# finlaymiller/torch-vae

Hardware: AMD Instinct MI355X
Metric: training samples/sec (VAE step: forward+ELBO+backward+AdamW), synthetic pianoroll (higher is better)
Workload: dtype bf16; 1 GPU; VanillaVAE latent_dim=16, 128x128 synthetic pianoroll, batch 256/GPU (generalised bottleneck 256*(H/16)^2); img_size=128, latent_dim=16, batch_per_gpu=256, global_batch=256, parallelism=dp1, optimizer=AdamW+OneCycle (encoder, decoder groups)

## Files before the change

### torch_vae_amd/csrc/conv_mfma.cuh

```cuda
#pragma once
#include "common.cuh"

enum { EPI_FWD = 0, EPI_BWD = 1, EPI_PLAIN = 2 };

template <typename T> struct ConvArgs {
    const T* src0; const T* src1; const float* coef; float slope;
    const T* wp; const float* bias;
    T* out;
    const T* yout; const float* ocoef; float oslope;
    double* stat;
    int B, Hs, Ws, Cin, Cout;
    int lth, ltw, lTB, tiles_x, tiles_y;
    int two_src, epi;
    unsigned m_pp, m_pw, m_tx, m_txy;
    long long* dbg;
    BnFuse fuse;
    int rev, n_mt;
    int xcd;
    T* stage_out;
};

__device__ __forceinline__ int fastdiv(int x, unsigned m) { return m ? (int)__umulhi((unsigned)x, m) : x; }
static inline unsigned fastdiv_magic(int d) { return d <= 1 ? 0u : (unsigned)((0x100000000ULL + (unsigned long long)d - 1) / (unsigned long long)d); }

// ... 1079 lines not shown
    sdl = wave_sum(sdl); bsum = wave_sum(bsum);
    __syncthreads();
    if (r < 9) {
#pragma unroll
        for (int i = 0; i < 16; ++i) red[wave][r * 32 + acc_row(i, lane)] = accw[i];
    }
    if (h == 0) { red[wave][288 + r] = s1; red[wave][320 + r] = s2; }
    if (lane == 0) { red[wave][352] = sdl; red[wave][353] = bsum; }
    __syncthreads();
    for (int j = tid; j < 288; j += 256) a.slab[(size_t)blockIdx.x * 288 + j] = red[0][j] + red[1][j] + red[2][j] + red[3][j];
    if (tid < 64) unsafeAtomicAdd(&a.stat[stat_rep() * 64 + tid], (double)(red[0][288 + tid] + red[1][288 + tid] + red[2][288 + tid] + red[3][288 + tid]));
    if (tid == 64) unsafeAtomicAdd(&a.accum[stat_rep() * 8 + 2], (double)(red[0][352] + red[1][352] + red[2][352] + red[3][352]));
    if (tid == 65) unsafeAtomicAdd(&a.accum[stat_rep() * 8 + 0], (double)(red[0][353] + red[1][353] + red[2][353] + red[3][353]));
}

template <typename T> struct DenseArgs {
    const T* A; const float* coef; float slope; int C;
    const T* Bp;
    float* slab;
    int M, K, Npad, ksteps_per_split;
    BnFuse fuse;
};

template <typename T, int NT>
__global__ __launch_bounds__(256) void dense_kernel(DenseArgs<T> a) {
    const int tid = threadIdx.x, lane = tid & 63, wave = tid >> 6, r = lane & 31, h = lane >> 5;
    const int m = blockIdx.x * 128 + wave * 32 + r, n0 = blockIdx.z * 32 * NT;
    const int ks0 = blockIdx.y * a.ksteps_per_split, ks1 = min(a.K / 16, ks0 + a.ksteps_per_split);
    __shared__ float dcf[2 * 256];
    if (a.coef) {
        const bool writer = blockIdx.x == 0 && blockIdx.y == 0 && blockIdx.z == 0;
        for (int c = tid; c < a.C; c += 256) {
            if (a.fuse.mode == BNF_FWD) { float k1; bn_fused_channel(a.fuse, c, writer, dcf[c], k1, dcf[256 + c]); }
            else { dcf[c] = a.coef[c]; dcf[256 + c] = a.coef[2 * a.C + c]; }
        }
        __syncthreads();
    }
    f32x16 acc[NT];
#pragma unroll
    for (int nt = 0; nt < NT; ++nt)
#pragma unroll
        for (int i = 0; i < 16; ++i) acc[nt][i] = 0.f;
    for (int ks = ks0; ks < ks1; ++ks) {
        const int k = ks * 16 + 8 * h;
        Frag<T> af;
        if (m < a.M) {
            Frag<T> raw = load_frag(a.A + (size_t)m * a.K + k);
            if (a.coef) {
#pragma unroll
                for (int j = 0; j < 8; ++j) {
                    const int c = (k + j) & (a.C - 1);
                    float v;
                    if constexpr (sizeof(T) == 4) v = raw.v[j]; else v = (float)raw.v[j];
                    af.set(j, leaky(v * dcf[c] + dcf[256 + c], a.slope));
                }
            } else {
                af = raw;
            }
        } else {
#pragma unroll
            for (int j = 0; j < 8; ++j) af.set(j, 0.f);
        }
#pragma unroll
        for (int nt = 0; nt < NT; ++nt) {
            const int n = n0 + nt * 32 + r;
            Frag<T> bf = load_frag(a.Bp + ((size_t)(k >> 3) * a.Npad + (n < a.Npad ? n : 0)) * 8);
            mma(acc[nt], af, bf);
        }
    }
#pragma unroll
    for (int nt = 0; nt < NT; ++nt)
#pragma unroll
        for (int i = 0; i < 16; ++i) {
            const int mm = blockIdx.x * 128 + wave * 32 + acc_row(i, lane), n = n0 + nt * 32 + r;
            if (mm < a.M && n < a.Npad) a.slab[((size_t)blockIdx.y * a.M + mm) * a.Npad + n] = acc[nt][i];
        }
}
```

### torch_vae_amd/csrc/edge_kernels.cuh

```cuda
#pragma once
#include "common.cuh"

__device__ __forceinline__ float cg_sum(float v) {
#pragma unroll
    for (int o = 4; o < 64; o <<= 1) v += __shfl_xor(v, o, 64);
    return v;
}

template <typename T> __device__ __forceinline__ void load8(const T* p, float* o);
template <> __device__ __forceinline__ void load8<float>(const float* p, float* o) {
    f32x4 a = *reinterpret_cast<const f32x4*>(p), b = *reinterpret_cast<const f32x4*>(p + 4);
#pragma unroll
    for (int i = 0; i < 4; ++i) { o[i] = a[i]; o[4 + i] = b[i]; }
}
template <> __device__ __forceinline__ void load8<bf16>(const bf16* p, float* o) {
    bf16x8 a = *reinterpret_cast<const bf16x8*>(p);
#pragma unroll
    for (int i = 0; i < 8; ++i) o[i] = (float)a[i];
}
template <> __device__ __forceinline__ void load8<f16>(const f16* p, float* o) {
    f16x8 a = *reinterpret_cast<const f16x8*>(p);
#pragma unroll
    for (int i = 0; i < 8; ++i) o[i] = (float)a[i];
}
// ... 750 lines not shown
#pragma unroll
            for (int u = 0; u < 8; ++u)
                av[u] = (bb + u < nb) ? leaky(tofloat(a.y[(size_t)(bc + bb + u) * a.F + fp]) * sc + sh, a.slope) : 0.f;
#pragma unroll
            for (int u = 0; u < 8; ++u)
#pragma unroll
                for (int q = 0; q < JT / 4; ++q) {
                    const f32x4 d = *reinterpret_cast<const f32x4*>(&dl_s[(bb + u) * JT + q * 4]);
#pragma unroll
                    for (int e = 0; e < 4; ++e) acc[q * 4 + e] += d[e] * av[u];
                }
        }
    }
#pragma unroll
    for (int j = 0; j < JT; ++j) {
        const int jj = j0 + j;
        const size_t zoff = (size_t)blockIdx.z * a.L * a.F;
        if (jj < a.L) a.dwmu[zoff + (size_t)jj * a.F + fr] = acc[j];
        else if (jj < L2) a.dwvar[zoff + (size_t)(jj - a.L) * a.F + fr] = acc[j];
    }
}

constexpr int DECIN_LC = 512;
static inline size_t decin_fwd_lds(int L) { return (size_t)16 * std::min(L, DECIN_LC) * 4; }
template <typename T>
__global__ __launch_bounds__(256) void decin_fwd_kernel(const float* __restrict__ z, const float* __restrict__ wd,
                                                        const float* __restrict__ bd, T* __restrict__ d0, int B, int F, int L, int s2) {
    constexpr int BT = 16;
    extern __shared__ __attribute__((aligned(16))) float z_s[];
    const int tid = threadIdx.x, fp = blockIdx.x * 256 + tid, b0 = blockIdx.y * BT, fr = fref_of(fp, s2);
    float acc[BT];
    const float bias = bd[fr];
#pragma unroll
    for (int bb = 0; bb < BT; ++bb) acc[bb] = bias;
    const float* wrow = wd + (size_t)fr * L;
    for (int l0 = 0; l0 < L; l0 += DECIN_LC) {
        const int nl = min(DECIN_LC, L - l0);
        if (l0) __syncthreads();
        for (int i = tid; i < BT * nl; i += 256) {
            const int bb = i / nl, l = i - bb * nl;
            z_s[i] = (b0 + bb < B) ? z[(size_t)(b0 + bb) * L + l0 + l] : 0.f;
        }
        __syncthreads();
        if ((L & 3) == 0) {
            for (int l = 0; l < nl; l += 4) {
                const f32x4 w = *reinterpret_cast<const f32x4*>(wrow + l0 + l);
#pragma unroll
                for (int bb = 0; bb < BT; ++bb) {
                    const f32x4 zz = *reinterpret_cast<const f32x4*>(&z_s[bb * nl + l]);
                    acc[bb] += zz[0] * w[0] + zz[1] * w[1] + zz[2] * w[2] + zz[3] * w[3];
                }
            }
        } else {
            for (int l = 0; l < nl; ++l) {
                const float w = wrow[l0 + l];
#pragma unroll
                for (int bb = 0; bb < BT; ++bb) acc[bb] += z_s[bb * nl + l] * w;
            }
        }
    }
#pragma unroll
    for (int bb = 0; bb < BT; ++bb)
        if (b0 + bb < B) d0[(size_t)(b0 + bb) * F + fp] = fromfloat<T>(acc[bb]);
}

template <typename T>
__global__ __launch_bounds__(256) void decin_wgrad_kernel(const T* __restrict__ dd0, const float* __restrict__ z,
                                                          float* __restrict__ dwd, float* __restrict__ dbd, int B, int F, int L, int s2,
                                                          int bsplit) {
    constexpr int LT = 32, BC = 64;
    __shared__ __attribute__((aligned(16))) float z_s[BC * LT];
    const int tid = threadIdx.x, l0 = blockIdx.y * LT;
    int fp, fr;
    fmap_ref_major(blockIdx.x, tid, s2, fp, fr);
    float acc[LT], sb = 0.f;
#pragma unroll
    for (int l = 0; l < LT; ++l) acc[l] = 0.f;
    const int bz0 = blockIdx.z * bsplit, bz1 = min(B, bz0 + bsplit);
    for (int bc = bz0; bc < bz1; bc += BC) {
        __syncthreads();
        for (int i = tid; i < BC * LT; i += 256) {
            const int bb = i / LT, l = i % LT;
            z_s[i] = (bc + bb < bz1 && l0 + l < L) ? z[(size_t)(bc + bb) * L + l0 + l] : 0.f;
        }
        __syncthreads();
        const int nb = min(BC, bz1 - bc);
// ... 137 lines not shown
```

### torch_vae_amd/csrc/latent_mfma.cuh

```cuda
#pragma once
#include "common.cuh"

struct FeatTile {
    int P, lP, CW, pix0, c0, s2;
    __device__ __forceinline__ FeatTile(int blk, int s2_) : s2(s2_) {
        P = s2_ < 8 ? s2_ : 8; lP = 31 - __clz(P); CW = 64 >> lP;
        const int lpb = (31 - __clz(s2_)) - lP;
        const int cblk = blk >> lpb; pix0 = (blk - (cblk << lpb)) << lP; c0 = cblk * CW;
    }
    __device__ __forceinline__ int fp(int col) const { return (pix0 + (col & (P - 1))) * 256 + c0 + (col >> lP); }
    __device__ __forceinline__ int fref(int col) const { return (c0 + (col >> lP)) * s2 + pix0 + (col & (P - 1)); }
    __device__ __forceinline__ int chan(int col) const { return c0 + (col >> lP); }
};

template <typename T>
__device__ __forceinline__ void stage_feat_tile_f32(const T* __restrict__ X, const FeatTile& t, int b0, int B, int F, const float* __restrict__ coef,
                                                    float slope, float* xs, int tid) {
    constexpr int E = 16 / sizeof(T);
    constexpr int vpr = 64 / E;
    const int lgpp = (6 - t.lP) - (E == 8 ? 3 : 2);
    for (int v = tid; v < 256 * vpr; v += 256) {
        const int row = v / vpr, j = v - row * vpr, p = j >> lgpp, g = j - (p << lgpp);
        const int b = b0 + row;
        float o[E];
        if (b < B) {
            const Vec16<T> raw = *reinterpret_cast<const Vec16<T>*>(X + (size_t)b * F + (t.pix0 + p) * 256 + t.c0 + g * E);
#pragma unroll
            for (int e = 0; e < E; ++e) {
                float x = raw.get(e);
                if (coef) { const int c = t.c0 + g * E + e; x = leaky(x * coef[c] + coef[2 * 256 + c], slope); }
                o[e] = x;
            }
        } else {
#pragma unroll
            for (int e = 0; e < E; ++e) o[e] = 0.f;
        }
#pragma unroll
        for (int e = 0; e < E; ++e) xs[row * 64 + (g * E + e) * t.P + p] = o[e];
    }
}

struct BatchGemmArgs {
    const void* X; const float* coef; float slope;
    const float* Y; int ldy, ncols;
    int ones_col;
    float* out0; float* out1; float* outb;
    float* colsum0; float* colsum1;
    int B, F, L, s2; float scale;
};

template <typename T, bool TRANSPOSED>
__global__ __launch_bounds__(256) void batch_gemm_kernel(BatchGemmArgs a) {
    constexpr int NBMAX = 9;
    extern __shared__ __attribute__((aligned(16))) char smem[];
    float* xs = reinterpret_cast<float*>(smem);
    float* ys = xs + 256 * 64;
    const int tid = threadIdx.x, lane = tid & 63, wave = tid >> 6, r = lane & 31, h = lane >> 5;
    const int fblk = wave & 1, khalf = wave >> 1;
    const FeatTile t(blockIdx.x, a.s2);
    const int ntot = a.ncols + (a.ones_col ? 1 : 0), nblk = (ntot + 31) / 32;
    f32x16 acc[NBMAX];
#pragma unroll
    for (int nb = 0; nb < NBMAX; ++nb)
#pragma unroll
        for (int i = 0; i < 16; ++i) acc[nb][i] = 0.f;
    for (int b0 = 0; b0 < a.B; b0 += 256) {
        __syncthreads();
        stage_feat_tile_f32<T>(reinterpret_cast<const T*>(a.X), t, b0, a.B, a.F, a.coef, a.slope, xs, tid);
#pragma unroll
        for (int nb = 0; nb < NBMAX; ++nb) {
            if (nb < nblk) {
                __syncthreads();
                if ((a.ldy & 3) == 0 && (a.ncols & 3) == 0) {
                    for (int i = tid; i < 256 * 8; i += 256) {
                        const int row = i >> 3, nq = (i & 7) * 4, n = nb * 32 + nq, b = b0 + row;
                        f32x4 v = {0.f, 0.f, 0.f, 0.f};
                        if (b < a.B) {
                            if (n < a.ncols) v = *reinterpret_cast<const f32x4*>(a.Y + (size_t)b * a.ldy + n);
                            else if (a.ones_col && n == a.ncols) v[0] = 1.f;
                        }
                        *reinterpret_cast<f32x4*>(ys + row * 32 + nq) = v;
                    }
                } else {
                    for (int i = tid; i < 256 * 32; i += 256) {
                        const int row = i >> 5, n = nb * 32 + (i & 31), b = b0 + row;
                        float v = 0.f;
                        if (b < a.B) v = n < a.ncols ? a.Y[(size_t)b * a.ldy + n] : ((a.ones_col && n == a.ncols) ? 1.f : 0.f);
                        ys[i] = v;
                    }
                }
                __syncthreads();
                if (blockIdx.x == 0 && a.colsum0) {
                    float s = 0.f;
                    for (int row = tid >> 5; row < 256; row += 8) s += ys[row * 32 + (tid & 31)];
                    float* cs = ys + 256 * 32;
                    cs[tid] = s;
                    __syncthreads();
                    const int n = nb * 32 + tid;
                    if (tid < 32 && n < a.ncols) {
                        float v = 0.f;
#pragma unroll
                        for (int g = 0; g < 8; ++g) v += cs[g * 32 + tid];
                        float* dst = n < a.L ? a.colsum0 + n : a.colsum1 + (n - a.L);
                        *dst = (b0 == 0 ? 0.f : *dst) + v * a.scale;
                    }
                }
                const float* xp = xs + (khalf * 128 + h) * 64 + fblk * 32 + r;
                const float* yp = ys + (khalf * 128 + h) * 32 + r;
#pragma unroll 8
                for (int s = 0; s < 64; ++s) {
                    const float xv = xp[s * 2 * 64], yv = yp[s * 2 * 32];
                    if constexpr (TRANSPOSED) acc[nb] = __builtin_amdgcn_mfma_f32_32x32x2f32(yv, xv, acc[nb], 0, 0, 0);
                    else acc[nb] = __builtin_amdgcn_mfma_f32_32x32x2f32(xv, yv, acc[nb], 0, 0, 0);
                }
// ... 11 lines not shown
    if (khalf == 0) {
#pragma unroll
        for (int nb = 0; nb < NBMAX; ++nb) {
            if (nb < nblk) {
#pragma unroll
                for (int i = 0; i < 16; ++i) {
                    const float v = (acc[nb][i] + red[((fblk * NBMAX + nb) * 16 + i) * 64 + lane]) * a.scale;
                    if constexpr (TRANSPOSED) {
                        const int n = nb * 32 + acc_row(i, lane), col = fblk * 32 + r;
                        if (n < a.ncols) {
                            float* dst = n < a.L ? a.out0 + (size_t)n * a.F : a.out1 + (size_t)(n - a.L) * a.F;
                            dst[t.fref(col)] = v;
                        }
                    } else {
                        const int col = fblk * 32 + acc_row(i, lane), n = nb * 32 + r;
                        if (n < a.ncols) a.out0[(size_t)t.fref(col) * a.L + n] = v;
                        else if (a.ones_col && n == a.ncols) a.outb[t.fref(col)] = v;
                    }
                }
            }
        }
    }
}
static inline size_t batch_gemm_lds() { return (size_t)(256 * 64 + 256 * 32 + 8 * 32) * 4; }

struct RowGemmArgs {
    const float* Y; int ldy, K;
    const float* Wf; const void* Wp; int npad;
    const float* bias;
    void* out;
    const void* y; const float* ocoef; float slope;
    const float* gpre; float gmul;
    double* stat;
    int B, F, s2;
};

template <typename T, int EPI>
__global__ __launch_bounds__(256) void row_gemm_kernel(RowGemmArgs a) {
    constexpr int KC = 32, YP = KC + 1;
    constexpr int E = 16 / sizeof(T);
    extern __shared__ __attribute__((aligned(16))) char smem[];
    float* ws = reinterpret_cast<float*>(smem);
    float* ys = ws + KC * 64;
    T* ot = reinterpret_cast<T*>(ys + 256 * YP);
    float* sred = reinterpret_cast<float*>(ot + 256 * 64);
    const int tid = threadIdx.x, lane = tid & 63, wave = tid >> 6, r = lane & 31, h = lane >> 5;
// ... 116 lines not shown
```

### torch_vae_amd/csrc/vae_api.hip

```cpp
#include <map>
#include <mutex>
#include "vae_ctx.h"
#include "edge_kernels.cuh"
#include "loglik.cuh"
#include "grad_clip.cuh"
#include "total_corr.cuh"

static thread_local std::string g_err;
int vae_set_error(const char* what, const char* why) {
    g_err = std::string(what) + ": " + why;
    return -1;
}

extern "C" const char* vae_last_error(void) { return g_err.c_str(); }
extern "C" int vae_abi_version(void) { return 1; }

static void param_shapes(int H, int L, int gen, int64_t* sizes) {
    const int s = gen ? H / 16 : 2;
    const int64_t F = 256LL * s * s;
    const int enc_ci[4] = {1, 32, 64, 128}, enc_co[4] = {32, 64, 128, 256};
    int k = 0;
    for (int i = 0; i < 4; ++i) { sizes[k++] = 9LL * enc_ci[i] * enc_co[i]; sizes[k++] = enc_co[i]; sizes[k++] = enc_co[i]; sizes[k++] = enc_co[i]; }
    sizes[k++] = L * F; sizes[k++] = L; sizes[k++] = L * F; sizes[k++] = L; sizes[k++] = F * L; sizes[k++] = F;
    const int dec_ci[3] = {256, 128, 64}, dec_co[3] = {128, 64, 32};
// ... 58 lines not shown
        (void)hipStreamSynchronize(c->comm);
        for (int i = 0; i < vae_ctx::NFORK; ++i) (void)hipEventDestroy(c->ev_fork[i]);
        (void)hipEventDestroy(c->ev_pack); (void)hipEventDestroy(c->ev_comm);
        if (c->ev_kl) (void)hipEventDestroy(c->ev_kl);
        for (int i = 0; i < vae_ctx::NBUCKET; ++i) (void)hipEventDestroy(c->ev_bucket[i]);
    }
    delete c;
}
extern "C" int64_t vae_workspace_bytes(const vae_ctx* c) { return c ? c->ws_bytes : 0; }

struct OptionDef { const char* name; int& (*ref)(vae_ctx&); int def; int (*norm)(int); };
static int opt_any(int v) { return v; }
static int opt_min1(int v) { return std::max(1, v); }
static int opt_fused_grid(int v) { return std::max(1, std::min(v, 512)); }
static int opt_max1024(int v) { return std::min(v, 1024); }
static int opt_max48(int v) { return std::min(v, 48); }
static int opt_fused_wgrad(int v) { return v == 1 ? 3 : v == 2 ? 1 : v == 3 ? 2 : 0; }
#define OPT(member, def, norm) {#member, [](vae_ctx& c) -> int& { return c.member; }, def, norm}
#define OPT_WK(member, def, norm) {"knob_wgrad_" #member, [](vae_ctx& c) -> int& { return c.wk.member; }, def, norm}
static const OptionDef kOptions[] = {
    OPT(use_tr16, 1, opt_any), OPT(use_mfma_convout, 1, opt_any), OPT(use_pipelined, 1, opt_any), OPT(use_side_stream, 1, opt_any),
    OPT(use_fused_bn, 1, opt_any), OPT(use_fused_convout, 1, opt_any), OPT(use_fused_wgrad, 1, opt_fused_wgrad), OPT(use_recomp_dz, 0, opt_any),
    OPT(use_raw_wgrad, 0, opt_any), OPT(use_deep, 1, opt_any), OPT(use_latent_mfma, 6, opt_any), OPT(use_convout_stream, 1, opt_any),
    OPT(use_dnf_stream, 1, opt_any), OPT(use_upf_stream, 1, opt_any), OPT(use_fc_dgrad8, 1, opt_any), OPT(use_wgrad_split, 1, opt_any),
    OPT(knob_up_per_cu, 2, opt_any), OPT(knob_down_per_cu, 2, opt_min1), OPT(knob_bwd_per_cu, 0, opt_any), OPT(knob_nt_max, 4, opt_any),
    OPT(knob_up_nt_max, 1, opt_min1), OPT(knob_wave_nt_max, 4, opt_any), OPT(knob_lay22_min_nt, 2, opt_any), OPT(knob_lay42, 1, opt_any),
    OPT(knob_down_waves, 8, opt_any), OPT(knob_pipe_max_cout, 256, opt_any), OPT(knob_xcd_map, 1, opt_any), OPT(knob_rev, 4, opt_any),
    OPT(knob_lean, 1, opt_any), OPT(knob_pack_grid, 128, opt_min1), OPT(knob_conv1_grid, 512, opt_any), OPT(knob_fused_grid, 256, opt_fused_grid),
    OPT(knob_convout_grid, 1536, opt_any), OPT(knob_convout_bwd_grid, 1024, opt_any), OPT(knob_convout_step_grid, 1024, opt_min1),
    OPT(knob_convout_bands, 0, opt_any), OPT(knob_wgrad_layer_wgs, 0, opt_any), OPT(knob_skip_wgrad, 0, opt_any), OPT(knob_ablate_b, 0, opt_any),
    OPT(knob_ablate_f, 0, opt_any),
    OPT_WK(tile, 1, opt_any), OPT_WK(wide, 1, opt_any), OPT_WK(mid8, 0, opt_any), OPT_WK(force_simple, 0, opt_any),
    OPT_WK(wgs, 128, opt_max1024), OPT_WK(wide_wgs, 128, opt_max1024), OPT_WK(cap_mb, 48, opt_max48),
};
#undef OPT_WK
#undef OPT
static const OptionDef* find_option(const char* name) {
    for (const OptionDef& o : kOptions) if (name && !strcmp(name, o.name)) return &o;
    return nullptr;
}

extern "C" vae_ctx* vae_create(int H, int L, int maxB, int dtype, int gen) {
    vae_ctx* c = new vae_ctx();
    c->H = H; c->L = L; c->maxB = maxB; c->dtype = dtype; c->gen = gen;
    for (const OptionDef& o : kOptions) o.ref(*c) = o.norm(o.def);
    if (getenv("VAE_NO_SIDE_STREAM")) c->use_side_stream = 0;
    if (vae_param_layout(H, L, gen, c->poff, c->psz, &c->ptotal) != 0) { delete c; return nullptr; }
// ... 777 lines not shown
```

### torch_vae_amd/csrc/vae_ctx.h

```cpp
#pragma once
#include <hip/hip_runtime.h>
#include <stdio.h>
#include <string.h>
#include <math.h>
#include <string>
#include <vector>
#include <algorithm>
#include <type_traits>

#include "../../include/vae_step.h"

int vae_set_error(const char* what, const char* why);

#include "common.cuh"

#define LAUNCH_CHECK(name)                                                        \
    do {                                                                          \
        hipError_t _e = hipGetLastError();                                        \
        if (_e != hipSuccess) return vae_set_error(name, hipGetErrorString(_e)); \
    } while (0)

template <typename K, typename... Args>
static int launch(const char* name, K kernel, dim3 grid, dim3 block, size_t lds_bytes, hipStream_t st, const Args&... args) {
    if (lds_bytes > 160 * 1024) return vae_set_error("lds", "tile needs more than 160 KiB LDS");
// ... 84 lines not shown
    PackDesc* d_descs; std::vector<PackDesc> h_descs; const float* packed_for = nullptr;
    float* slab; size_t slab_floats;
    static constexpr int NSIDE = 3, NFORK = 16;
    hipStream_t side[NSIDE]; float* side_slab[NSIDE]; hipEvent_t ev_fork[NFORK], ev_join[NSIDE], ev_pack; int side_rr = 0, fork_rr = 0, n_side_ok = 0;
    static constexpr int NBUCKET = 2; hipEvent_t ev_bucket[NBUCKET];
    hipStream_t comm; hipEvent_t ev_comm; int comm_busy = 0;
    void* nccl_comm = nullptr; int comm_rank = 0, comm_world = 0;
    double* dstats; size_t n_dstats; double* accum;
    float* reduce_tmp = nullptr; size_t reduce_tmp_floats = 0; unsigned reduce_slot = 0;
    float* fused_slab[3] = {nullptr, nullptr, nullptr}; size_t fused_slab_floats = 0;
    static constexpr int KL_SIDE = 2;
    void* kl_ws = nullptr; unsigned* kl_tk = nullptr; hipEvent_t ev_kl = nullptr;
    unsigned long long* kl_d() const { return static_cast<unsigned long long*>(kl_ws); }
    double* kl_scal() const { return reinterpret_cast<double*>(kl_d() + L); }
    float* kl_factor() const { return reinterpret_cast<float*>(kl_scal() + 2); }
    const double* kl_shaped() const { return fwd.kl_kind != VAE_KL_PLAIN ? kl_scal() : nullptr; }
    void* tc_ws = nullptr; size_t tc_ws_bytes = 0; int tc_ws_B = 0;
    float* tc_grad() const { return static_cast<float*>(tc_ws); }
    double* ps_part = nullptr; int ps_tb = 0, ps_ntile = 0;
    float* ll_f = nullptr; double* ll_part = nullptr; double* ll_lat = nullptr;
    double* ll_kb = nullptr; size_t ll_kb_n = 0;
    std::vector<void*> allocs; int64_t ws_bytes = 0;
    int use_tr16, use_mfma_convout, use_pipelined, use_side_stream, use_fused_bn, use_fused_convout, use_fused_wgrad, use_recomp_dz, use_raw_wgrad,
        use_deep, use_latent_mfma, use_convout_stream, use_dnf_stream, use_upf_stream, use_fc_dgrad8, use_wgrad_split;
    int knob_up_per_cu, knob_down_per_cu, knob_bwd_per_cu, knob_nt_max, knob_up_nt_max, knob_wave_nt_max, knob_lay22_min_nt, knob_lay42,
        knob_down_waves, knob_pipe_max_cout, knob_xcd_map, knob_rev, knob_lean, knob_pack_grid, knob_conv1_grid, knob_fused_grid,
        knob_convout_grid, knob_convout_bwd_grid, knob_convout_step_grid, knob_convout_bands, knob_wgrad_layer_wgs,
        knob_skip_wgrad, knob_ablate_b, knob_ablate_f;
    WgradKnobs wk;
    int recon = VAE_RECON_BCE, kl_kind = VAE_KL_PLAIN; double kl_param = 0.0; double recon_param = 0.0;
    FwdRecord fwd;
    long long* dbg_buf = nullptr; char dbg_tag[32] = {0}; int dbg_epi = 0;
    int prof = 0; const char* tag = nullptr; struct ProfRec { std::string name; hipEvent_t e0, e1; double bytes, flops; int side; int launches = 1; }; std::vector<ProfRec> prof_recs;
    hipStream_t cur_stream = nullptr; bool cur_stream_set = false;
};

struct ProfScope {
    vae_ctx* c; hipStream_t st; int idx;
    ProfScope(vae_ctx* c_, const char* name, double bytes, double flops, hipStream_t st_) : c(c_), st(st_), idx(-1) {
        if (!c || !c->prof) return;
        vae_ctx::ProfRec r; r.name = std::string(name) + (c->tag ? std::string(" @") + c->tag : std::string()); r.bytes = bytes; r.flops = flops;
        r.side = (c->cur_stream_set && st != c->cur_stream) ? 1 : 0;
        if (hipEventCreate(&r.e0) != hipSuccess || hipEventCreate(&r.e1) != hipSuccess) return;
        (void)hipEventRecord(r.e0, st);
        c->prof_recs.push_back(r); idx = (int)c->prof_recs.size() - 1;
    }
    ~ProfScope() { if (idx >= 0) (void)hipEventRecord(c->prof_recs[idx].e1, st); }
// ... 95 lines not shown
```

### torch_vae_amd/csrc/vae_impl.cuh

```cuda
#pragma once
#include "vae_ctx.h"
#include "conv_mfma.cuh"
#include "conv_pipe.cuh"
#include "edge_kernels.cuh"
#include "conv_fused.cuh"
#include "conv_deep.cuh"
#include "latent_mfma.cuh"
#include "convout_stream.cuh"
#include "wgrad_split.cuh"
#include "upfinal_stream.cuh"
#include "dnfirst_stream.cuh"
#include "grad_paths.cuh"

template <typename F> static int pick_recon(vae_ctx* c, F&& f) {
    return pick_const<VAE_RECON_BCE, VAE_RECON_MSE, VAE_RECON_WBCE>("reconstruction term", c->fwd.recon, f);
}
template <typename F> static int pick_recon_per_sample(vae_ctx* c, F&& f) {
    return pick_const<VAE_RECON_BCE, VAE_RECON_MSE>("reconstruction term", c->fwd.recon == VAE_RECON_WBCE ? VAE_RECON_BCE : c->fwd.recon, f);
}

static int stream_bands(int B, int rows, int max_bands, int min_rows, int rows_per_tick, int fixed_ticks) {
    const int ncu = 256;
    long best = -1; int nb = 1;
    for (int cand = 1; cand <= max_bands && rows / cand >= min_rows; cand *= 2) {
// ... 234 lines not shown
                a.dbg = (c->dbg_buf && c->tag && !strcmp(c->tag, c->dbg_tag) && c->dbg_epi == 32) ? c->dbg_buf : nullptr;
                rc = pick_bool(convt, [&](auto C) { return go(wgrad_split_kernel<T, decltype(C)::value>, 1024, wgrad_split_lds<T>(npix)); });
            }
            else if (WA == 4 && raw) rc = go(wgrad_kernel<T, 4, 1, false, true, 8, true>, 512, lds);
            else if (WA == 4) rc = pick_bool(convt, [&](auto C) { return go(wgrad_kernel<T, 4, 1, decltype(C)::value, true, 8>, 512, lds); });
            else rc = pick_bool(convt, [&](auto C) { return go(wgrad_kernel<T, 2, 1, decltype(C)::value, true, 8>, 512, lds); });
        }
        else rc = vae_set_error("wgrad", "eight-wave tiles need 16-bit storage");
    }
    else {
        const auto tile = [&](auto A, auto B_) { return pick_bool(convt, [&](auto C) { return pick_bool(pre, [&](auto P) {
            return go(wgrad_kernel<T, decltype(A)::value, decltype(B_)::value, decltype(C)::value, decltype(P)::value>, 256, lds); }); }); };
        using one = std::integral_constant<int, 1>; using two = std::integral_constant<int, 2>;
        if (WA == 2 && WB == 2) rc = tile(two{}, two{});
        else if (WA == 2 && WB == 1) rc = tile(two{}, one{});
        else if (WA == 1 && WB == 1) rc = tile(one{}, one{});
        else rc = vae_set_error("wgrad", "no kernel variant for this channel tile");
    }
    if (rc) return -1;
    }
    return launch_reduce(slab_buf, nsplit, (size_t)9 * a.CA * a.CB, dw_out, a.CA, a.CB, st, c);
}

template <typename T>
static int launch_dense(vae_ctx* c, DenseArgs<T> a, int* nsplit_out, hipStream_t st) {
    const int nb = a.Npad / 32, NT = nb % 4 == 0 ? 4 : (nb % 2 == 0 ? 2 : 1);
    if (a.Npad % 32) return vae_set_error("dense", "Npad must be a multiple of 32");
    const int mt = (a.M + 127) / 128, ntile = a.Npad / (32 * NT), ksteps = a.K / 16;
    int nsplit = std::max(1, std::min(ksteps, 512 / std::max(1, mt * ntile)));
    a.ksteps_per_split = (ksteps + nsplit - 1) / nsplit;
    nsplit = (ksteps + a.ksteps_per_split - 1) / a.ksteps_per_split;
    if ((size_t)nsplit * a.M * a.Npad > c->slab_floats) return vae_set_error("dense", "slab too small");
    a.slab = c->slab;
    dim3 grid(mt, nsplit, ntile);
    *nsplit_out = nsplit;
    ProfScope ps(c, "dense(fc / decoder_input dgrad)", sizeof(T) * ((double)a.M * a.K + (double)a.K * a.Npad), 2.0 * a.M * a.K * a.Npad, st);
    return pick_const<1, 2, 4>("dense_kernel", NT, [&](auto N) { return launch("dense_kernel", dense_kernel<T, decltype(N)::value>, grid, dim3(256), 0, st, a); });
}
template <typename T>
int pack_weights(vae_ctx* c, const float* params, hipStream_t st) {
    std::vector<PackDesc>& d = c->h_descs;
    if (c->packed_for != params || d.empty()) {
        d.clear();
        const int ci[8] = {1, 32, 64, 128, 256, 128, 64, 32}, co[8] = {32, 64, 128, 256, 128, 64, 32, 32};
        for (int i = 1; i < 8; ++i) {
            const bool conv = i < 4;
            PackDesc p; memset(&p, 0, sizeof(p));
            p.src = params + c->poff[c->lay[i].p_convw]; p.kind = 0; p.n = 9L * ci[i] * co[i];
            p.A = conv ? co[i] : ci[i]; p.Bc = conv ? ci[i] : co[i];
            p.dst = c->wp_fwd[i]; p.k_is_first = conv ? 0 : 1; d.push_back(p);
            p.dst = c->wp_dg[i]; p.k_is_first = conv ? 1 : 0; d.push_back(p);
        }
        PackDesc p; memset(&p, 0, sizeof(p));
        p.kind = 1; p.src = params + c->poff[16]; p.src2 = params + c->poff[18]; p.dst = c->fcpack; p.npad = c->npad_fc; p.L = c->L; p.s2 = c->s2; p.n = c->F * c->npad_fc; d.push_back(p);
        p.kind = 2; p.src = params + c->poff[20]; p.src2 = nullptr; p.dst = c->dipack; p.npad = c->npad_di; p.n = c->F * c->npad_di; d.push_back(p);
        p.kind = 3; p.src = params + c->poff[38]; p.dst = c->wout_t; p.A = 32; p.n = 288; d.push_back(p);
        HIP_CHECK_RET(hipMemcpyAsync(c->d_descs, d.data(), d.size() * sizeof(PackDesc), hipMemcpyHostToDevice, st));
        c->packed_for = params;
    }
    ProfScope ps(c, "pack_weights", 0, 0, st);
// ... 67 lines not shown
            c->ps_ntile = (H / 8) * (H / 32);
            const dim3 grid(std::min(m.n_tiles, c->knob_convout_grid));
            return pick_recon_per_sample(c, [&](auto R) { return launch("convout_fwd_mfma_kernel(per sample)", convout_fwd_mfma_kernel<T, decltype(R)::value, true>, grid, dim3(256), 0, st, m); });
        }
    }
    c->ps_ntile = (H / 16) * (H / 32);
    const dim3 grid(B * (H / 16) * (H / 32));
    return pick_recon_per_sample(c, [&](auto R) { return launch("convout_fwd_kernel(per sample)", convout_fwd_kernel<T, decltype(R)::value, true>, grid, dim3(256), 0, st, a); });
}

template <typename T>
int decode_impl(vae_ctx* c, const float* z, int B, const float* params, float* bn_running, int64_t* nbt, int train,
                       const float* x, float* xhat, hipStream_t st) {
    const int H = c->H, L = c->L;
    c->tag = "latent";
    {
        ProfScope ps(c, "decin_fwd", (double)sizeof(T) * B * (double)c->F + 4.0 * c->F * L, 2.0 * B * c->F * L, st);
        if (c->use_latent_mfma & 1) {
            RowGemmArgs g; memset(&g, 0, sizeof(g));
            g.Y = z; g.ldy = L; g.K = L; g.Wf = params + c->poff[20]; g.bias = params + c->poff[21]; g.out = c->d0; g.B = B; g.F = (int)c->F; g.s2 = c->s2;
            if (launch("row_gemm_kernel", row_gemm_kernel<T, 0>, dim3((unsigned)(c->F / 64)), dim3(256), row_gemm_lds<T>(), st, g)) return -1;
        } else {
            dim3 grid((unsigned)(c->F / 256), (B + 15) / 16);
            if (launch("decin_fwd_kernel", decin_fwd_kernel<T>, grid, dim3(256), decin_fwd_lds(L), st, z, params + c->poff[20], params + c->poff[21],
                       reinterpret_cast<T*>(c->d0), B, (int)c->F, L, c->s2)) return -1;
        }
    }
    for (int i = 4; i < 8; ++i) {
        c->tag = kLayerTag[i];
        ConvArgs<T> a; memset(&a, 0, sizeof(a));
        if (i == 4) { a.src0 = reinterpret_cast<const T*>(c->d0); a.coef = c->ident; a.slope = 1.f; a.Cin = 256; }
        else { a.src0 = reinterpret_cast<const T*>(c->lay[i - 1].y); a.coef = c->lay[i - 1].block; a.slope = kSlope; a.Cin = c->lay[i - 1].C; }
        a.wp = reinterpret_cast<const T*>(c->wp_fwd[i]); a.bias = params + c->poff[c->lay[i].p_convb];
        a.out = reinterpret_cast<T*>(c->lay[i].y); a.stat = c->lay[i].stat_f;
        a.B = B; a.Hs = c->lay[i].H / 2; a.Ws = c->lay[i].W / 2; a.Cout = c->lay[i].C; a.epi = EPI_FWD;
        if (i > 4 && input_bn_fwd(c, i - 1, params, bn_running, nbt, train, will_pipe(c, a), &a.fuse, st)) return -1;
        if (i == 5) {
            c->lay[4].act_ok = 0;
            if (train && c->lay[4].act && raw_wgrad_ok<T>(c, 5) && will_pipe(c, a)) { a.stage_out = reinterpret_cast<T*>(c->lay[4].act); c->lay[4].act_ok = 1; }
        }
        if (launch_up<T>(c, a, st)) return -1;
    }
    c->tag = "final_layer.3";
    {
        ConvOutArgs a;
        a.yf = c->lay[7].y; a.coef = c->lay[7].block; a.wt = c->wout_t; a.bias = params + c->poff[39]; a.target = x;
        a.xhat = xhat; a.dlogit = c->dlogit; a.accum = c->accum; a.B = B; a.H = H; a.W = H;
        a.inv_n = (float)(1.0 / ((double)B * H * H)); a.slope = kSlope; a.recon_w = (float)c->fwd.recon_param; a.part = nullptr; a.tB = 0;
// ... 309 lines not shown
    return 0;
}

template <typename T>
static int backward_second(vae_ctx* c, const float* x, const float* params, float* grads, const float* gscale,
                           const float* g_mu, const float* g_lv, const float* g_z, const float* g_pre, float kld_weight, int add_kl,
                           hipStream_t st, int mode = 0, float* out = nullptr) {
    const int B = c->fwd.B, H = c->H, L = c->L;
    const int nz = std::max(1, std::min(8, B / 8)), bsplit = (B + nz - 1) / nz;
    c->tag = "latent";
    {
        const bool lat_mfma = (c->use_latent_mfma & 4) && 2 * L <= 9 * 32;
        if (mode != 1) {
            const bool mfma = (c->use_latent_mfma & 2) && L + 1 <= 9 * 32;
            SideFork f = fork_side(c, st);
            if (f.rc) return f.rc;
            float* sw = f.slab; float* sb = f.slab + (size_t)nz * c->F * L;
            {
                ProfScope ps(c, "decin_wgrad", (double)sizeof(T) * B * (double)c->F + 4.0 * c->F * L, 2.0 * B * c->F * L, f.st);
                if (mfma) {
                    BatchGemmArgs g; memset(&g, 0, sizeof(g));
                    g.X = c->dd0; g.coef = nullptr; g.slope = 1.f; g.Y = c->fwd.z; g.ldy = L; g.ncols = L; g.ones_col = 1;
                    g.out0 = grads + c->poff[20]; g.outb = grads + c->poff[21]; g.B = B; g.F = (int)c->F; g.L = L; g.s2 = c->s2; g.scale = c->fwd.ginv;
                    if (launch("batch_gemm_kernel", batch_gemm_kernel<T, false>, dim3((unsigned)(c->F / 64)), dim3(256), batch_gemm_lds(), f.st, g)) return -1;
                } else {
                    dim3 grid((unsigned)(c->F / 256), (L + 31) / 32, nz);
                    if (launch("decin_wgrad_kernel", decin_wgrad_kernel<T>, grid, dim3(256), 0, f.st, reinterpret_cast<const T*>(c->dd0), c->fwd.z, sw, sb, B, (int)c->F, L, c->s2, bsplit)) return -1;
                }
            }
            if (!mfma) {
                if (launch_reduce(sw, nz, (size_t)c->F * L, grads + c->poff[20], 0, 0, f.st, c)) return -1;
                if (launch_reduce(sb, nz, (size_t)c->F, grads + c->poff[21], 0, 0, f.st, c)) return -1;
            }
        }
        int nsplit = 0;
        if (mode == 0 || (mode == 2 && out)) {
            DenseArgs<T> a; memset(&a, 0, sizeof(a));
            a.A = reinterpret_cast<const T*>(c->dd0); a.coef = nullptr; a.slope = 1.f; a.C = 256;
            a.Bp = reinterpret_cast<const T*>(c->dipack); a.M = B; a.K = (int)c->F; a.Npad = c->npad_di;
            if (launch_dense<T>(c, a, &nsplit, st)) return -1;
        }
        if (mode == 2) {
            if (!out) return join_sides(c, st);
            ProfScope ps(c, "latent_dz", 4.0 * nsplit * B * L + 4.0 * B * L, 0, st);
            if (launch("latent_dz_kernel", latent_dz_kernel, dim3((B * L + 255) / 256), dim3(256), 0, st, c->slab, nsplit, c->npad_di, B, L, c->fwd.ginv, out)) return -1;
            return join_sides(c, st);
        }
// ... 9 lines not shown
        } else if (add_kl && c->fwd.kl_kind != VAE_KL_PLAIN) {
            if (join_kl(c, st)) return -1;
            lb.factor = c->kl_factor();
            if (latent_bwd(latent_bwd_kernel<true>)) return -1;
        } else if (latent_bwd(latent_bwd_kernel<false>)) return -1;
        if (!lat_mfma) {
            SideFork f = fork_side(c, st);
            if (f.rc) return f.rc;
            if (launch("colsum_kernel", colsum_kernel, dim3(2 * L), dim3(64), 0, f.st, c->dlat, B, 2 * L, grads + c->poff[17], grads + c->poff[19], L, c->fwd.ginv)) return -1;
        }
    }
    {
        const bool mfma = (c->use_latent_mfma & 4) && 2 * L <= 9 * 32;
        SideFork f = fork_side(c, st);
        if (f.rc) return f.rc;
        float* smu = f.slab; float* svar = f.slab + (size_t)nz * L * c->F;
        {
            ProfScope ps(c, "fc_wgrad", (double)sizeof(T) * B * (double)c->F + 8.0 * c->F * L, 4.0 * B * c->F * L, f.st);
            if (mfma) {
                BatchGemmArgs g; memset(&g, 0, sizeof(g));
                g.X = c->lay[3].y; g.coef = c->lay[3].block; g.slope = kSlope; g.Y = c->dlat; g.ldy = 2 * L; g.ncols = 2 * L; g.ones_col = 0;
                g.out0 = grads + c->poff[16]; g.out1 = grads + c->poff[18]; g.colsum0 = grads + c->poff[17]; g.colsum1 = grads + c->poff[19];
                g.B = B; g.F = (int)c->F; g.L = L; g.s2 = c->s2; g.scale = c->fwd.ginv;
                if (launch("batch_gemm_kernel", batch_gemm_kernel<T, true>, dim3((unsigned)(c->F / 64)), dim3(256), batch_gemm_lds(), f.st, g)) return -1;
            } else {
                FcWgradArgs<T> w;
                w.dlat = c->dlat; w.y = reinterpret_cast<const T*>(c->lay[3].y); w.coef = c->lay[3].block; w.slope = kSlope;
                w.B = B; w.F = (int)c->F; w.L = L; w.s2 = c->s2; w.bsplit = bsplit; w.dwmu = smu; w.dwvar = svar;
                if (launch("fc_wgrad_kernel", fc_wgrad_kernel<T>, dim3((unsigned)(c->F / 256), (2 * L + 31) / 32, nz), dim3(256), 0, f.st, w)) return -1;
            }
        }
        if (!mfma) {
            if (launch_reduce(smu, nz, (size_t)L * c->F, grads + c->poff[16], 0, 0, f.st, c)) return -1;
            if (launch_reduce(svar, nz, (size_t)L * c->F, grads + c->poff[18], 0, 0, f.st, c)) return -1;
        }
    }
    {
        ProfScope ps(c, "fc_dgrad", (double)sizeof(T) * (2.0 * B * c->F + 2.0 * c->F * L), 4.0 * B * c->F * L, st);
        if ((c->use_latent_mfma & 8) && 2 * L <= 256) {
            RowGemmArgs g; memset(&g, 0, sizeof(g));
            g.Y = c->dlat; g.ldy = 2 * L; g.K = 2 * L; g.Wp = c->fcpack; g.npad = c->npad_fc; g.out = c->lay[3].dz;
            g.y = c->lay[3].y; g.ocoef = c->lay[3].block; g.slope = kSlope; g.gpre = g_pre; g.gmul = c->fwd.gmul; g.stat = c->lay[3].stat_b;
            g.B = B; g.F = (int)c->F; g.s2 = c->s2;
            if (launch("row_gemm_kernel", row_gemm_kernel<T, 1>, dim3((unsigned)(c->F / 64)), dim3(256), row_gemm_lds<T>(), st, g)) return -1;
        } else {
            FcDgradArgs<T> d;
            d.dlat = c->dlat; d.wp = reinterpret_cast<const T*>(c->fcpack); d.npad = c->npad_fc; d.y = reinterpret_cast<const T*>(c->lay[3].y);
// ... 103 lines not shown
```

Baseline: 234,400 samples/s.

## Keep more global loads in flight in latent dense, batch-GEMM and decoder-input kernels

Adds a default-on use_latent_inflight option that changes three latent-layer kernels. dense_kernel gains a register ring that prefetches several k-steps of A and B fragments ahead of the MFMAs. batch_gemm_kernel loads feature and Y tiles into registers before staging them to LDS and prefetches the next Y block. decin_fwd_kernel stages its output through LDS so it can issue 16-byte coalesced stores. The aim is to hide global memory latency in these small GEMMs, at the cost of more registers and LDS, which may lower occupancy.

```diff
diff --git a/torch_vae_amd/csrc/conv_mfma.cuh b/torch_vae_amd/csrc/conv_mfma.cuh
--- a/torch_vae_amd/csrc/conv_mfma.cuh
+++ b/torch_vae_amd/csrc/conv_mfma.cuh
@@ -1125,7 +1125,7 @@
     BnFuse fuse;
 };
 
-template <typename T, int NT>
+template <typename T, int NT, bool INFLIGHT>
 __global__ __launch_bounds__(256) void dense_kernel(DenseArgs<T> a) {
     const int tid = threadIdx.x, lane = tid & 63, wave = tid >> 6, r = lane & 31, h = lane >> 5;
     const int m = blockIdx.x * 128 + wave * 32 + r, n0 = blockIdx.z * 32 * NT;
@@ -1144,11 +1144,10 @@
     for (int nt = 0; nt < NT; ++nt)
 #pragma unroll
         for (int i = 0; i < 16; ++i) acc[nt][i] = 0.f;
-    for (int ks = ks0; ks < ks1; ++ks) {
+    const auto a_operand = [&](const Frag<T>& raw, int ks) {
         const int k = ks * 16 + 8 * h;
         Frag<T> af;
         if (m < a.M) {
-            Frag<T> raw = load_frag(a.A + (size_t)m * a.K + k);
             if (a.coef) {
 #pragma unroll
                 for (int j = 0; j < 8; ++j) {
@@ -1164,11 +1163,43 @@
 #pragma unroll
             for (int j = 0; j < 8; ++j) af.set(j, 0.f);
         }
-#pragma unroll
-        for (int nt = 0; nt < NT; ++nt) {
-            const int n = n0 + nt * 32 + r;
-            Frag<T> bf = load_frag(a.Bp + ((size_t)(k >> 3) * a.Npad + (n < a.Npad ? n : 0)) * 8);
-            mma(acc[nt], af, bf);
+        return af;
+    };
+    const auto b_ptr = [&](int ks, int nt) {
+        const int k = ks * 16 + 8 * h, n = n0 + nt * 32 + r;
+        return a.Bp + ((size_t)(k >> 3) * a.Npad + (n < a.Npad ? n : 0)) * 8;
+    };
+    if constexpr (INFLIGHT) {
+        constexpr int PER = (1 + NT) * (sizeof(T) == 4 ? 8 : 4), DEPTH = 128 / PER > 8 ? 8 : (128 / PER < 2 ? 2 : 128 / PER);
+        Frag<T> ar[DEPTH], br[DEPTH][NT];
+        const T* arow = a.A + (size_t)min(m, a.M - 1) * a.K + 8 * h;
+        const auto request = [&](int d, int ks) {
+            ar[d] = load_frag(arow + ks * 16);
+#pragma unroll
+            for (int nt = 0; nt < NT; ++nt) br[d][nt] = load_frag(b_ptr(ks, nt));
+        };
+#pragma unroll
+        for (int d = 0; d < DEPTH; ++d)
+            if (ks0 + d < ks1) request(d, ks0 + d);
+        for (int kb = ks0; kb < ks1; kb += DEPTH) {
+#pragma unroll
+            for (int d = 0; d < DEPTH; ++d) {
+                const int ks = kb + d;
+                if (ks < ks1) {
+                    const Frag<T> af = a_operand(ar[d], ks);
+#pragma unroll
+                    for (int nt = 0; nt < NT; ++nt) mma(acc[nt], af, br[d][nt]);
+                    if (ks + DEPTH < ks1) request(d, ks + DEPTH);
+                }
+            }
+        }
+    } else {
+        for (int ks = ks0; ks < ks1; ++ks) {
+            Frag<T> raw;
+            if (m < a.M) raw = load_frag(a.A + (size_t)m * a.K + ks * 16 + 8 * h);
+            const Frag<T> af = a_operand(raw, ks);
+#pragma unroll
+            for (int nt = 0; nt < NT; ++nt) mma(acc[nt], af, load_frag(b_ptr(ks, nt)));
         }
     }
 #pragma unroll
diff --git a/torch_vae_amd/csrc/edge_kernels.cuh b/torch_vae_amd/csrc/edge_kernels.cuh
--- a/torch_vae_amd/csrc/edge_kernels.cuh
+++ b/torch_vae_amd/csrc/edge_kernels.cuh
@@ -796,8 +796,8 @@
 }
 
 constexpr int DECIN_LC = 512;
-static inline size_t decin_fwd_lds(int L) { return (size_t)16 * std::min(L, DECIN_LC) * 4; }
-template <typename T>
+static inline size_t decin_fwd_lds(int L, size_t out_tile_elem_bytes = 0) { return (size_t)16 * std::min(L, DECIN_LC) * 4 + 16 * 256 * out_tile_elem_bytes; }
+template <typename T, bool VIA_LDS>
 __global__ __launch_bounds__(256) void decin_fwd_kernel(const float* __restrict__ z, const float* __restrict__ wd,
                                                         const float* __restrict__ bd, T* __restrict__ d0, int B, int F, int L, int s2) {
     constexpr int BT = 16;
@@ -833,9 +833,23 @@
             }
         }
     }
-#pragma unroll
-    for (int bb = 0; bb < BT; ++bb)
-        if (b0 + bb < B) d0[(size_t)(b0 + bb) * F + fp] = fromfloat<T>(acc[bb]);
+    if constexpr (VIA_LDS) {
+        constexpr int E = 16 / sizeof(T), VPR = 256 / E;
+        T* o_s = reinterpret_cast<T*>(z_s + BT * min(L, DECIN_LC));
+#pragma unroll
+        for (int bb = 0; bb < BT; ++bb) o_s[bb * 256 + tid] = fromfloat<T>(acc[bb]);
+        __syncthreads();
+#pragma unroll
+        for (int i = 0; i < BT * VPR / 256; ++i) {
+            const int v = tid + i * 256, bb = v / VPR, q = v - bb * VPR;
+            if (b0 + bb < B)
+                *reinterpret_cast<Vec16<T>*>(d0 + (size_t)(b0 + bb) * F + blockIdx.x * 256 + q * E) = *reinterpret_cast<const Vec16<T>*>(o_s + bb * 256 + q * E);
+        }
+    } else {
+#pragma unroll
+        for (int bb = 0; bb < BT; ++bb)
+            if (b0 + bb < B) d0[(size_t)(b0 + bb) * F + fp] = fromfloat<T>(acc[bb]);
+    }
 }
 
 template <typename T>
diff --git a/torch_vae_amd/csrc/latent_mfma.cuh b/torch_vae_amd/csrc/latent_mfma.cuh
--- a/torch_vae_amd/csrc/latent_mfma.cuh
+++ b/torch_vae_amd/csrc/latent_mfma.cuh
@@ -40,6 +40,81 @@
     }
 }
 
+struct BatchGemmArgs;
+__host__ __device__ static inline bool batch_gemm_yvec(const BatchGemmArgs& a);
+
+template <typename T> struct FeatTileRegs {
+    static constexpr int E = 16 / sizeof(T), vpr = 64 / E, NV = vpr, RSTEP = 256 / vpr;
+    Vec16<T> raw[NV];
+    float sc[E], sh[E];
+    int row0, p, g;
+    __device__ __forceinline__ void init(const FeatTile& t, const float* __restrict__ coef, int tid) {
+        const int lgpp = (6 - t.lP) - (E == 8 ? 3 : 2);
+        const int j = tid & (vpr - 1);
+        row0 = tid / vpr; p = j >> lgpp; g = j - (p << lgpp);
+        if (coef) {
+#pragma unroll
+            for (int e = 0; e < E; ++e) { const int c = t.c0 + g * E + e; sc[e] = coef[c]; sh[e] = coef[2 * 256 + c]; }
+        }
+    }
+    __device__ __forceinline__ void load(const T* __restrict__ X, const FeatTile& t, int b0, int B, int F) {
+        const T* src = X + (t.pix0 + p) * 256 + t.c0 + g * E;
+#pragma unroll
+        for (int i = 0; i < NV; ++i) raw[i] = *reinterpret_cast<const Vec16<T>*>(src + (size_t)min(b0 + row0 + i * RSTEP, B - 1) * F);
+    }
+    __device__ __forceinline__ void store(const FeatTile& t, int b0, int B, bool has_coef, float slope, float* xs) const {
+#pragma unroll
+        for (int i = 0; i < NV; ++i) {
+            const int row = row0 + i * RSTEP;
+            const bool live = b0 + row < B;
+#pragma unroll
+            for (int e = 0; e < E; ++e) {
+                float x = raw[i].get(e);
+                if (has_coef) x = leaky(x * sc[e] + sh[e], slope);
+                xs[row * 64 + (g * E + e) * t.P + p] = live ? x : 0.f;
+            }
+        }
+    }
+};
+
+struct YTileRegs {
+    float v[32];
+    float fill;
+    bool incol;
+    __device__ __forceinline__ void load(const float* __restrict__ Y, int ldy, int ncols, int ones_col, bool vec, int nb, int b0, int B, int tid) {
+        const int n = nb * 32 + (vec ? (tid & 7) * 4 : (tid & 31));
+        incol = n < ncols; fill = (ones_col && n == ncols) ? 1.f : 0.f;
+        const float* src = Y + (incol ? n : 0);
+        if (vec) {
+#pragma unroll
+            for (int i = 0; i < 8; ++i) {
+                const f32x4 q = *reinterpret_cast<const f32x4*>(src + (size_t)min(b0 + (tid >> 3) + i * 32, B - 1) * ldy);
+#pragma unroll
+                for (int e = 0; e < 4; ++e) v[i * 4 + e] = q[e];
+            }
+        } else {
+#pragma unroll
+            for (int i = 0; i < 32; ++i) v[i] = src[(size_t)min(b0 + (tid >> 5) + i * 8, B - 1) * ldy];
+        }
+    }
+    __device__ __forceinline__ void store(bool vec, int b0, int B, float* ys, int tid) const {
+        if (vec) {
+#pragma unroll
+            for (int i = 0; i < 8; ++i) {
+                const int row = (tid >> 3) + i * 32;
+                const bool live = b0 + row < B;
+                f32x4 q;
+#pragma unroll
+                for (int e = 0; e < 4; ++e) q[e] = live ? (incol ? v[i * 4 + e] : (e == 0 ? fill : 0.f)) : 0.f;
+                *reinterpret_cast<f32x4*>(ys + row * 32 + (tid & 7) * 4) = q;
+            }
+        } else {
+#pragma unroll
+            for (int i = 0; i < 32; ++i) ys[tid + i * 256] = (b0 + (tid >> 5) + i * 8 < B) ? (incol ? v[i] : fill) : 0.f;
+        }
+    }
+};
+
 struct BatchGemmArgs {
     const void* X; const float* coef; float slope;
     const float* Y; int ldy, ncols;
@@ -49,7 +124,7 @@
     int B, F, L, s2; float scale;
 };
 
-template <typename T, bool TRANSPOSED>
+template <typename T, bool TRANSPOSED, bool INFLIGHT, bool YVEC = false>
 __global__ __launch_bounds__(256) void batch_gemm_kernel(BatchGemmArgs a) {
     constexpr int NBMAX = 9;
     extern __shared__ __attribute__((aligned(16))) char smem[];
@@ -64,14 +139,27 @@
     for (int nb = 0; nb < NBMAX; ++nb)
 #pragma unroll
         for (int i = 0; i < 16; ++i) acc[nb][i] = 0.f;
+    const bool yvec = INFLIGHT ? YVEC : batch_gemm_yvec(a);
+    FeatTileRegs<T> xr;
+    if constexpr (INFLIGHT) xr.init(t, a.coef, tid);
     for (int b0 = 0; b0 < a.B; b0 += 256) {
         __syncthreads();
-        stage_feat_tile_f32<T>(reinterpret_cast<const T*>(a.X), t, b0, a.B, a.F, a.coef, a.slope, xs, tid);
+        YTileRegs yr;
+        if constexpr (INFLIGHT) {
+            xr.load(reinterpret_cast<const T*>(a.X), t, b0, a.B, a.F);
+            yr.load(a.Y, a.ldy, a.ncols, a.ones_col, YVEC, 0, b0, a.B, tid);
+            __builtin_amdgcn_sched_barrier(0);
+            xr.store(t, b0, a.B, a.coef != nullptr, a.slope, xs);
+        } else {
+            stage_feat_tile_f32<T>(reinterpret_cast<const T*>(a.X), t, b0, a.B, a.F, a.coef, a.slope, xs, tid);
+        }
 #pragma unroll
         for (int nb = 0; nb < NBMAX; ++nb) {
             if (nb < nblk) {
-                __syncthreads();
-                if ((a.ldy & 3) == 0 && (a.ncols & 3) == 0) {
+                if (!INFLIGHT || nb) __syncthreads();
+                if constexpr (INFLIGHT) {
+                    yr.store(YVEC, b0, a.B, ys, tid);
+                } else if (yvec) {
                     for (int i = tid; i < 256 * 8; i += 256) {
                         const int row = i >> 3, nq = (i & 7) * 4, n = nb * 32 + nq, b = b0 + row;
                         f32x4 v = {0.f, 0.f, 0.f, 0.f};
@@ -90,6 +178,9 @@
                     }
                 }
                 __syncthreads();
+                if constexpr (INFLIGHT) {
+                    if (nb + 1 < nblk) yr.load(a.Y, a.ldy, a.ncols, a.ones_col, YVEC, nb + 1, b0, a.B, tid);
+                }
                 if (blockIdx.x == 0 && a.colsum0) {
                     float s = 0.f;
                     for (int row = tid >> 5; row < 256; row += 8) s += ys[row * 32 + (tid & 31)];
@@ -147,6 +238,7 @@
         }
     }
 }
+__host__ __device__ static inline bool batch_gemm_yvec(const BatchGemmArgs& a) { return (a.ldy & 3) == 0 && (a.ncols & 3) == 0; }
 static inline size_t batch_gemm_lds() { return (size_t)(256 * 64 + 256 * 32 + 8 * 32) * 4; }
 
 struct RowGemmArgs {
diff --git a/torch_vae_amd/csrc/vae_api.hip b/torch_vae_amd/csrc/vae_api.hip
--- a/torch_vae_amd/csrc/vae_api.hip
+++ b/torch_vae_amd/csrc/vae_api.hip
@@ -104,7 +104,7 @@
     OPT(use_tr16, 1, opt_any), OPT(use_mfma_convout, 1, opt_any), OPT(use_pipelined, 1, opt_any), OPT(use_side_stream, 1, opt_any),
     OPT(use_fused_bn, 1, opt_any), OPT(use_fused_convout, 1, opt_any), OPT(use_fused_wgrad, 1, opt_fused_wgrad), OPT(use_recomp_dz, 0, opt_any),
     OPT(use_raw_wgrad, 0, opt_any), OPT(use_deep, 1, opt_any), OPT(use_latent_mfma, 6, opt_any), OPT(use_convout_stream, 1, opt_any),
-    OPT(use_dnf_stream, 1, opt_any), OPT(use_upf_stream, 1, opt_any), OPT(use_fc_dgrad8, 1, opt_any), OPT(use_wgrad_split, 1, opt_any),
+    OPT(use_dnf_stream, 1, opt_any), OPT(use_upf_stream, 1, opt_any), OPT(use_fc_dgrad8, 1, opt_any), OPT(use_wgrad_split, 1, opt_any), OPT(use_latent_inflight, 1, opt_any),
     OPT(knob_up_per_cu, 2, opt_any), OPT(knob_down_per_cu, 2, opt_min1), OPT(knob_bwd_per_cu, 0, opt_any), OPT(knob_nt_max, 4, opt_any),
     OPT(knob_up_nt_max, 1, opt_min1), OPT(knob_wave_nt_max, 4, opt_any), OPT(knob_lay22_min_nt, 2, opt_any), OPT(knob_lay42, 1, opt_any),
     OPT(knob_down_waves, 8, opt_any), OPT(knob_pipe_max_cout, 256, opt_any), OPT(knob_xcd_map, 1, opt_any), OPT(knob_rev, 4, opt_any),
diff --git a/torch_vae_amd/csrc/vae_ctx.h b/torch_vae_amd/csrc/vae_ctx.h
--- a/torch_vae_amd/csrc/vae_ctx.h
+++ b/torch_vae_amd/csrc/vae_ctx.h
@@ -130,7 +130,7 @@
     double* ll_kb = nullptr; size_t ll_kb_n = 0;
     std::vector<void*> allocs; int64_t ws_bytes = 0;
     int use_tr16, use_mfma_convout, use_pipelined, use_side_stream, use_fused_bn, use_fused_convout, use_fused_wgrad, use_recomp_dz, use_raw_wgrad,
-        use_deep, use_latent_mfma, use_convout_stream, use_dnf_stream, use_upf_stream, use_fc_dgrad8, use_wgrad_split;
+        use_deep, use_latent_mfma, use_latent_inflight, use_convout_stream, use_dnf_stream, use_upf_stream, use_fc_dgrad8, use_wgrad_split;
     int knob_up_per_cu, knob_down_per_cu, knob_bwd_per_cu, knob_nt_max, knob_up_nt_max, knob_wave_nt_max, knob_lay22_min_nt, knob_lay42,
         knob_down_waves, knob_pipe_max_cout, knob_xcd_map, knob_rev, knob_lean, knob_pack_grid, knob_conv1_grid, knob_fused_grid,
         knob_convout_grid, knob_convout_bwd_grid, knob_convout_step_grid, knob_convout_bands, knob_wgrad_layer_wgs,
diff --git a/torch_vae_amd/csrc/vae_impl.cuh b/torch_vae_amd/csrc/vae_impl.cuh
--- a/torch_vae_amd/csrc/vae_impl.cuh
+++ b/torch_vae_amd/csrc/vae_impl.cuh
@@ -280,6 +280,13 @@
     return launch_reduce(slab_buf, nsplit, (size_t)9 * a.CA * a.CB, dw_out, a.CA, a.CB, st, c);
 }
 
+template <typename T, bool TRANSPOSED>
+static int launch_batch_gemm(vae_ctx* c, const BatchGemmArgs& g, hipStream_t st) {
+    const auto go = [&](auto kernel) { return launch("batch_gemm_kernel", kernel, dim3((unsigned)(c->F / 64)), dim3(256), batch_gemm_lds(), st, g); };
+    if (!c->use_latent_inflight) return go(batch_gemm_kernel<T, TRANSPOSED, false>);
+    return pick_bool(batch_gemm_yvec(g), [&](auto V) { return go(batch_gemm_kernel<T, TRANSPOSED, true, decltype(V)::value>); });
+}
+
 template <typename T>
 static int launch_dense(vae_ctx* c, DenseArgs<T> a, int* nsplit_out, hipStream_t st) {
     const int nb = a.Npad / 32, NT = nb % 4 == 0 ? 4 : (nb % 2 == 0 ? 2 : 1);
@@ -293,7 +300,8 @@
     dim3 grid(mt, nsplit, ntile);
     *nsplit_out = nsplit;
     ProfScope ps(c, "dense(fc / decoder_input dgrad)", sizeof(T) * ((double)a.M * a.K + (double)a.K * a.Npad), 2.0 * a.M * a.K * a.Npad, st);
-    return pick_const<1, 2, 4>("dense_kernel", NT, [&](auto N) { return launch("dense_kernel", dense_kernel<T, decltype(N)::value>, grid, dim3(256), 0, st, a); });
+    return pick_const<1, 2, 4>("dense_kernel", NT, [&](auto N) { return pick_bool(c->use_latent_inflight != 0, [&](auto I) {
+        return launch("dense_kernel", dense_kernel<T, decltype(N)::value, decltype(I)::value>, grid, dim3(256), 0, st, a); }); });
 }
 template <typename T>
 int pack_weights(vae_ctx* c, const float* params, hipStream_t st) {
@@ -407,8 +415,10 @@
             if (launch("row_gemm_kernel", row_gemm_kernel<T, 0>, dim3((unsigned)(c->F / 64)), dim3(256), row_gemm_lds<T>(), st, g)) return -1;
         } else {
             dim3 grid((unsigned)(c->F / 256), (B + 15) / 16);
-            if (launch("decin_fwd_kernel", decin_fwd_kernel<T>, grid, dim3(256), decin_fwd_lds(L), st, z, params + c->poff[20], params + c->poff[21],
-                       reinterpret_cast<T*>(c->d0), B, (int)c->F, L, c->s2)) return -1;
+            if (pick_bool(c->use_latent_inflight != 0, [&](auto I) {
+                    constexpr bool via_lds = decltype(I)::value;
+                    return launch("decin_fwd_kernel", decin_fwd_kernel<T, via_lds>, grid, dim3(256), decin_fwd_lds(L, via_lds ? sizeof(T) : 0), st, z,
+                                  params + c->poff[20], params + c->poff[21], reinterpret_cast<T*>(c->d0), B, (int)c->F, L, c->s2); })) return -1;
         }
     }
     for (int i = 4; i < 8; ++i) {
@@ -764,7 +774,7 @@
                     BatchGemmArgs g; memset(&g, 0, sizeof(g));
                     g.X = c->dd0; g.coef = nullptr; g.slope = 1.f; g.Y = c->fwd.z; g.ldy = L; g.ncols = L; g.ones_col = 1;
                     g.out0 = grads + c->poff[20]; g.outb = grads + c->poff[21]; g.B = B; g.F = (int)c->F; g.L = L; g.s2 = c->s2; g.scale = c->fwd.ginv;
-                    if (launch("batch_gemm_kernel", batch_gemm_kernel<T, false>, dim3((unsigned)(c->F / 64)), dim3(256), batch_gemm_lds(), f.st, g)) return -1;
+                    if (launch_batch_gemm<T, false>(c, g, f.st)) return -1;
                 } else {
                     dim3 grid((unsigned)(c->F / 256), (L + 31) / 32, nz);
                     if (launch("decin_wgrad_kernel", decin_wgrad_kernel<T>, grid, dim3(256), 0, f.st, reinterpret_cast<const T*>(c->dd0), c->fwd.z, sw, sb, B, (int)c->F, L, c->s2, bsplit)) return -1;
@@ -820,7 +830,7 @@
                 g.X = c->lay[3].y; g.coef = c->lay[3].block; g.slope = kSlope; g.Y = c->dlat; g.ldy = 2 * L; g.ncols = 2 * L; g.ones_col = 0;
                 g.out0 = grads + c->poff[16]; g.out1 = grads + c->poff[18]; g.colsum0 = grads + c->poff[17]; g.colsum1 = grads + c->poff[19];
                 g.B = B; g.F = (int)c->F; g.L = L; g.s2 = c->s2; g.scale = c->fwd.ginv;
-                if (launch("batch_gemm_kernel", batch_gemm_kernel<T, true>, dim3((unsigned)(c->F / 64)), dim3(256), batch_gemm_lds(), f.st, g)) return -1;
+                if (launch_batch_gemm<T, true>(c, g, f.st)) return -1;
             } else {
                 FcWgradArgs<T> w;
                 w.dlat = c->dlat; w.y = reinterpret_cast<const T*>(c->lay[3].y); w.coef = c->lay[3].block; w.slope = kSlope;
```

Result: slower. 227,900 samples/s (-2.8%).
